# zhaoshan2/pangu-pytorch

Hardware: AMD Instinct MI355X
Metric: forward steps/sec (721x1440x13pl) per MI355X (higher is better)
Workload: dtype f32; 1 GPU; PanguModel fp32 forward, 1 sample/GPU, input (1,5,13,721,1440)+(1,4,721,1440), depths 2-6-6-2, dims 192/384, random-init weights (BASELINE configs[1]); parallelism=dp1

## Files before the change

### include/pangu_hip.h

```cpp
#ifndef PANGU_HIP_H
#define PANGU_HIP_H

#include <stdint.h>

#ifdef __cplusplus
extern "C" {
#endif

#define PANGU_ABI_VERSION 1

#define PANGU_OK 0
#define PANGU_E_SHAPE (-1)
#define PANGU_E_NULL (-2)
#define PANGU_E_DTYPE (-3)
#define PANGU_E_ARG (-4)
#define PANGU_E_RANGE (-5)

#define PANGU_F32 0
#define PANGU_BF16 1

#define PANGU_ACT_NONE 0
#define PANGU_ACT_GELU 1
#define PANGU_ACT_GELU_BWD 2
#define PANGU_ACT_ADD 3
#define PANGU_ACT_GELU_BWD_H 4

typedef void* pangu_stream_t;

int pangu_abi_version(void);
const char* pangu_error_string(int code);


int pangu_window_index_export(pangu_stream_t stream, int32_t* out, int Z, int H, int W, int shifted);

int pangu_window_mask_export(pangu_stream_t stream, float* out, int Z, int H, int W);


int pangu_linear_fwd(pangu_stream_t stream, const float* A, int lda, const float* W, const float* bias,
                     float* C, int ldc, int M, int N, int K, int act, float* aux);

int pangu_split_weight_bf16x3(pangu_stream_t stream, const float* W, int N, int K, void* image);
int pangu_linear_fwd_split(pangu_stream_t stream, const float* A, int lda, const void* image, const float* bias,
                           float* C, int ldc, int M, int N, int K, int act);

int pangu_linear_wgrad(pangu_stream_t stream, const float* dC, int lddc, const float* A, int lda, float* dW,
                       float* db, int M, int N, int K);
int pangu_linear_wgrad_ws(pangu_stream_t stream, const float* dC, int lddc, const float* A, int lda, float* dW,
                          float* db, int M, int N, int K, float* workspace, long long workspace_bytes);


int pangu_lora_wgrad_f32(pangu_stream_t stream, const float* dY, int lddy, const float* X, int ldx, const float* A,
                         const float* B, float* dA, float* dB, int M, int N, int K, int r, float scaling, float* workspace,
                         long long workspace_bytes);
int pangu_lora_wgrad_bf16(pangu_stream_t stream, const void* dY, int lddy, const void* X, int ldx, const float* A, const float* B,
                          float* dA, float* dB, int M, int N, int K, int r, float scaling, float* workspace,
                          long long workspace_bytes);
int pangu_lora_merge_f32(pangu_stream_t stream, const float* W, const float* A, const float* B, float* W_eff, int N, int K,
                         int r, float scaling);


int pangu_lora_dropout_fwd_f32(pangu_stream_t stream, const float* X, int ldx, float* Y, int ldy, const float* A, const float* B,
                               int M, int N, int K, int r, float scaling, double p, unsigned seed, int act, float* H, int ldh);
int pangu_lora_wgrad_dropout_f32(pangu_stream_t stream, const float* dY, int lddy, const float* X, int ldx, const float* A,
                                 const float* B, float* dA, float* dB, float* V, int M, int N, int K, int r, float scaling, double p,
                                 unsigned seed, float* workspace, long long workspace_bytes);
int pangu_lora_dropout_dx_f32(pangu_stream_t stream, float* dX, int lddx, const float* V, const float* A, int M, int K, int r,
                              double p, unsigned seed, const float* pre, int ldpre);


int pangu_lora_dropout_fwd_bf16(pangu_stream_t stream, const void* X, int ldx, void* Y, int ldy, const float* A, const float* B,
                                int M, int N, int K, int r, float scaling, double p, unsigned seed, int act, void* H, int ldh);
int pangu_lora_wgrad_dropout_bf16(pangu_stream_t stream, const void* dY, int lddy, const void* X, int ldx, const float* A,
                                  const float* B, float* dA, float* dB, float* V, int M, int N, int K, int r, float scaling, double p,
                                  unsigned seed, float* workspace, long long workspace_bytes);
int pangu_lora_dropout_dx_bf16(pangu_stream_t stream, void* dX, int lddx, const float* V, const float* A, int M, int K, int r,
                               double p, unsigned seed, const void* pre, int ldpre);


int pangu_window_attn_fwd(pangu_stream_t stream, const float* qkv, const float* qkv_bias, const float* esb,
                          float* out, float* lse, int Z, int H, int W, int C, int heads, int shifted);
int pangu_window_attn_fwd_compact(pangu_stream_t stream, const float* qkv, const float* qkv_bias,
                                  const float* esb_compact, float* out, float* lse, int Z, int H, int W, int C,
                                  int heads, int shifted);

int pangu_attn_windows_fwd(pangu_stream_t stream, const float* qkv, const float* esb, const float* mask,
                           long long mask_lon_stride, float* out, int n_lon, int types, int heads, int C);

int pangu_attn_windows_bwd(pangu_stream_t stream, const float* qkv, const float* esb, const float* mask,
                           long long mask_lon_stride, const float* dout, float* dqkv, float* d_esb, int n_lon, int types,
                           int heads, int C);

int pangu_window_attn_bwd(pangu_stream_t stream, const float* qkv, const float* qkv_bias, const float* esb,
                          const float* out, const float* lse, const float* dout, float* dqkv, float* dqkv_bias,
                          float* d_esb, int Z, int H, int W, int C, int heads, int shifted);


int pangu_ln_residual_fwd(pangu_stream_t stream, const float* y, const float* shortcut, int lds,
                          const float* gamma, const float* beta, float* out, int ldo, float* mean_rstd,
                          int N, int C, float branch_scale);

int pangu_linear_ln_residual_fwd(pangu_stream_t stream, const float* A, int lda, const float* W, const float* bias,
                                 const float* shortcut, int lds, const float* gamma, const float* beta, float* out, int ldo,
                                 int M, int N, int K, float branch_scale);

int pangu_ln_residual_bwd(pangu_stream_t stream, const float* dout, int lddo, const float* y, const float* gamma,
                          float* dy, float* dgamma, float* dbeta, int N, int C, float branch_scale);

int pangu_downsample_ln_fwd(pangu_stream_t stream, const float* x, int ldx, const float* gamma,
                            const float* beta, float* out, float* mean_rstd, int Z, int H, int W, int C);

int pangu_downsample_ln_bwd(pangu_stream_t stream, const float* dout, const float* x, int ldx, const float* gamma,
                            float* dx, float* dgamma, float* dbeta, int Z, int H, int W, int C, const float* dx_add);

int pangu_upsample_ln_fwd(pangu_stream_t stream, const float* y, const float* gamma, const float* beta,
                          float* out, float* mean_rstd, int Z, int H2, int W2, int H, int Co);

int pangu_upsample_ln_bwd(pangu_stream_t stream, const float* dout, const float* y, const float* gamma, float* dy,
                          float* dgamma, float* dbeta, int Z, int H2, int W2, int H, int Co);


int pangu_patch_embed_gather(pangu_stream_t stream, const float* input, const float* input_surface,
                             const float* surface_mean, const float* surface_std, const float* upper_mean,
                             const float* upper_std, const float* maps, const float* const_h,
                             float* a_surface, float* a_upper, int LAT, int LON, int levels_reversed);

int pangu_patch_embed_gather_bwd(pangu_stream_t stream, const float* da_surface, const float* da_upper,
                                 const float* surface_std, const float* upper_std, float* d_input,
                                 float* d_input_surface, int LAT, int LON, int levels_reversed);

int pangu_patch_recover_scatter(pangu_stream_t stream, const float* y_upper, const float* y_surface,
                                float* output, float* output_surface, int LAT, int LON);
int pangu_patch_recover_scatter_denorm(pangu_stream_t stream, const float* y_upper, const float* y_surface, float* output,
                                       float* output_surface, float* phys, float* phys_surface, const float* upper_mean,
                                       const float* upper_std, const float* surface_mean, const float* surface_std, int LAT,
                                       int LON);

int pangu_patch_recover_gather_bwd(pangu_stream_t stream, const float* d_output, const float* d_output_surface,
                                   float* dy_upper, float* dy_surface, int LAT, int LON);


int pangu_lat_weighted_sums(pangu_stream_t stream, const float* pred, const float* target, const float* lat_weight,
                            float* out, int planes, int H, int W);


int pangu_ensemble_perturb_f32(pangu_stream_t stream, float* upper, long long upper_member_stride, float* surface,
                               long long surface_member_stride, int E, int first_member, int H, int W, const float* amplitude,
                               const float* upper_std, const float* surface_std, unsigned int seed, int octaves, int period,
                               float persistence, int control);

int pangu_ensemble_stats_f32(pangu_stream_t stream, const float* members, long long member_stride, int E, const float* target,
                             const float* clim, const float* lat_weight, float* out, float* mean_out, float* std_out,
                             float* workspace, long long workspace_bytes, int planes, int H, int W);


int pangu_linear_fwd_bf16(pangu_stream_t stream, const void* A, int lda, const void* W, const float* bias, void* C,
                          int ldc, int M, int N, int K, int act, void* aux, int out_dtype);

int pangu_window_attn_fwd_bf16(pangu_stream_t stream, const void* qkv, const void* qkv_bias, const void* esb, void* out,
                               float* lse, int Z, int H, int W, int C, int heads, int shifted);

int pangu_window_attn_qkv_fwd_bf16(pangu_stream_t stream, const void* x, int ldx, const void* w_qkv, const float* b_qkv,
                                   const void* esb, void* out, float* lse, int Z, int H, int W, int C, int heads,
                                   int shifted);

int pangu_ln_residual_fwd_bf16(pangu_stream_t stream, const void* y, const void* shortcut, int lds, const float* gamma,
                               const float* beta, void* out, int ldo, int N, int C, float branch_scale);
int pangu_linear_ln_residual_fwd_bf16(pangu_stream_t stream, const void* A, int lda, const void* W, const float* bias,
                                      const void* shortcut, const float* gamma, const float* beta, void* out, int ldo, int M,
                                      int N, int K);
int pangu_mlp_ln_residual_fwd_bf16(pangu_stream_t stream, const void* x, int ldx, const void* w_packed, const float* b1,
                                   const float* b2, const float* gamma, const float* beta, void* out, int ldo, int M,
                                   int C, float branch_scale);
int pangu_mlp_ln_residual_train_fwd_bf16(pangu_stream_t stream, const void* x, int ldx, const void* w_packed,
                                         const float* b1, const float* b2, const float* gamma, const float* beta, void* out,
                                         int ldo, void* pre, int ldp, void* m, int ldm, int M, int C, float branch_scale);
int pangu_linear_gelu_bwd_bf16(pangu_stream_t stream, const void* A, int lda, const void* W, void* dpre, int ldc, int M,
                               int N, int K, const void* pre, void* h);
int pangu_downsample_ln_fwd_bf16(pangu_stream_t stream, const void* x, int ldx, const float* gamma, const float* beta,
                                 void* out, int Z, int H, int W, int C);
int pangu_upsample_ln_fwd_bf16(pangu_stream_t stream, const void* y, const float* gamma, const float* beta, void* out,
                               int Z, int H2, int W2, int H, int Co);

int pangu_patch_embed_gather_bf16(pangu_stream_t stream, const float* input, const float* input_surface,
                                  const float* surface_mean, const float* surface_std, const float* upper_mean,
                                  const float* upper_std, const float* maps, const float* const_h, void* a_surface,
                                  void* a_upper, int LAT, int LON, int levels_reversed);
// ... 70 lines not shown
```

### pangu-pytorch_amd/_lib.py

```python
import ctypes
import os
import re

_HERE = os.path.dirname(os.path.abspath(__file__))
LIB_PATH = os.environ.get("PANGU_HIP_LIB") or os.path.join(_HERE, "libpangu_hip.so")
HEADER_PATH = os.path.join(os.path.dirname(_HERE), "include", "pangu_hip.h")

_c = ctypes
_P, _I, _F = _c.c_void_p, _c.c_int, _c.c_float

SIGNATURES = {
    "pangu_abi_version": [],
    "pangu_error_string": [_I],
    "pangu_window_index_export": [_P, _P, _I, _I, _I, _I],
    "pangu_window_mask_export": [_P, _P, _I, _I, _I],
    "pangu_linear_fwd": [_P, _P, _I, _P, _P, _P, _I, _I, _I, _I, _I, _P],
    "pangu_split_weight_bf16x3": [_P, _P, _I, _I, _P],
    "pangu_linear_fwd_split": [_P, _P, _I, _P, _P, _P, _I, _I, _I, _I, _I],
    "pangu_linear_wgrad": [_P, _P, _I, _P, _I, _P, _P, _I, _I, _I],
    "pangu_linear_wgrad_ws": [_P, _P, _I, _P, _I, _P, _P, _I, _I, _I, _P, _c.c_longlong],
    "pangu_lora_wgrad_f32": [_P, _P, _I, _P, _I, _P, _P, _P, _P, _I, _I, _I, _I, _F, _P, _c.c_longlong],
    "pangu_lora_wgrad_bf16": [_P, _P, _I, _P, _I, _P, _P, _P, _P, _I, _I, _I, _I, _F, _P, _c.c_longlong],
    "pangu_lora_merge_f32": [_P, _P, _P, _P, _P, _I, _I, _I, _F],
    "pangu_lora_dropout_fwd_f32": [_P, _P, _I, _P, _I, _P, _P, _I, _I, _I, _I, _F, _c.c_double, _c.c_uint, _I, _P, _I],
    "pangu_lora_wgrad_dropout_f32": [_P, _P, _I, _P, _I, _P, _P, _P, _P, _P, _I, _I, _I, _I, _F, _c.c_double, _c.c_uint, _P,
                                     _c.c_longlong],
    "pangu_lora_dropout_dx_f32": [_P, _P, _I, _P, _P, _I, _I, _I, _c.c_double, _c.c_uint, _P, _I],
    "pangu_lora_dropout_fwd_bf16": [_P, _P, _I, _P, _I, _P, _P, _I, _I, _I, _I, _F, _c.c_double, _c.c_uint, _I, _P, _I],
    "pangu_lora_wgrad_dropout_bf16": [_P, _P, _I, _P, _I, _P, _P, _P, _P, _P, _I, _I, _I, _I, _F, _c.c_double, _c.c_uint, _P,
                                      _c.c_longlong],
    "pangu_lora_dropout_dx_bf16": [_P, _P, _I, _P, _P, _I, _I, _I, _c.c_double, _c.c_uint, _P, _I],
    "pangu_window_attn_bwd": [_P] * 10 + [_I] * 6,
    "pangu_ln_residual_bwd": [_P, _P, _I, _P, _P, _P, _P, _P, _I, _I, _F],
    "pangu_downsample_ln_bwd": [_P, _P, _P, _I, _P, _P, _P, _P, _I, _I, _I, _I, _P],
    "pangu_upsample_ln_bwd": [_P, _P, _P, _P, _P, _P, _P, _I, _I, _I, _I, _I],
    "pangu_patch_recover_gather_bwd": [_P, _P, _P, _P, _P, _I, _I],
    "pangu_lat_weighted_sums": [_P, _P, _P, _P, _P, _I, _I, _I],
    "pangu_ensemble_perturb_f32": [_P, _P, _c.c_longlong, _P, _c.c_longlong, _I, _I, _I, _I, _P, _P, _P, _c.c_uint, _I, _I, _F, _I],
    "pangu_ensemble_stats_f32": [_P, _P, _c.c_longlong, _I, _P, _P, _P, _P, _P, _P, _P, _c.c_longlong, _I, _I, _I],
    "pangu_linear_fwd_bf16": [_P, _P, _I, _P, _P, _P, _I, _I, _I, _I, _I, _P, _I],
    "pangu_window_attn_fwd_bf16": [_P, _P, _P, _P, _P, _P, _I, _I, _I, _I, _I, _I],
    "pangu_window_attn_qkv_fwd_bf16": [_P, _P, _I, _P, _P, _P, _P, _P, _I, _I, _I, _I, _I, _I],
    "pangu_ln_residual_fwd_bf16": [_P, _P, _P, _I, _P, _P, _P, _I, _I, _I, _F],
    "pangu_linear_ln_residual_fwd_bf16": [_P, _P, _I, _P, _P, _P, _P, _P, _P, _I, _I, _I, _I],
    "pangu_mlp_ln_residual_fwd_bf16": [_P, _P, _I, _P, _P, _P, _P, _P, _P, _I, _I, _I, _F],
    "pangu_mlp_ln_residual_train_fwd_bf16": [_P, _P, _I, _P, _P, _P, _P, _P, _P, _I, _P, _I, _P, _I, _I, _I, _F],
    "pangu_linear_gelu_bwd_bf16": [_P, _P, _I, _P, _P, _I, _I, _I, _I, _P, _P],
    "pangu_downsample_ln_fwd_bf16": [_P, _P, _I, _P, _P, _P, _I, _I, _I, _I],
    "pangu_upsample_ln_fwd_bf16": [_P, _P, _P, _P, _P, _I, _I, _I, _I, _I],
    "pangu_patch_embed_gather_bf16": [_P] * 11 + [_I, _I, _I],
    "pangu_linear_wgrad_bf16": [_P, _P, _I, _P, _I, _P, _P, _I, _I, _I],
    "pangu_linear_wgrad_bf16_ws": [_P, _P, _I, _P, _I, _P, _P, _I, _I, _I, _P, _c.c_longlong],
    "pangu_shadow_refresh_bf16": [_P, _P, _I, _c.c_longlong],
    "pangu_adam_step_multi": [_P, _P, _I, _c.c_longlong] + [_c.c_double] * 5 + [_F, _F],
    "pangu_grad_sumsq_multi": [_P, _P, _I, _c.c_longlong, _P],
    "pangu_grad_clip_state": [_P, _P, _c.c_longlong, _P, _I, _c.c_double, _c.c_double, _I],
    "pangu_adam_step_multi_scaled": [_P, _P, _I, _c.c_longlong] + [_c.c_double] * 5 + [_F, _F, _P],
    "pangu_weighted_l1_loss_blocks": [_I, _I, _c.c_longlong, _I, _c.c_longlong, _I],
    "pangu_weighted_l1_loss_fwd": [_P] * 9 + [_I, _I, _c.c_longlong, _I, _c.c_longlong, _I, _I] + [_P] * 4,
    "pangu_weighted_l1_loss_bwd": [_P] * 10 + [_I, _I, _c.c_longlong, _I, _c.c_longlong, _I, _I] + [_P] * 4,
    "pangu_rollout_l1_seed_bwd": [_P] * 14 + [_I, _I, _c.c_longlong, _I, _c.c_longlong, _I, _I] + [_P] * 4,
    "pangu_fair_crps_loss_blocks": [_I] * 7,
    "pangu_fair_crps_loss_fwd": [_P, _P, _P, _I] + [_P] * 7 + [_I] * 7 + [_P] * 4,
    "pangu_fair_crps_loss_bwd": [_P, _P, _P, _I] + [_P] * 8 + [_I] * 7 + [_P] * 4,
    "pangu_host_copy": [_P, _P, _c.c_longlong, _I],
    "pangu_window_attn_bwd_bf16": [_P] * 10 + [_I] * 6,
    "pangu_ln_residual_bwd_bf16": [_P, _P, _I, _P, _P, _P, _P, _P, _I, _I, _F],
    "pangu_downsample_ln_bwd_bf16": [_P, _P, _P, _I, _P, _P, _P, _P, _I, _I, _I, _I, _P],
    "pangu_upsample_ln_bwd_bf16": [_P, _P, _P, _P, _P, _P, _P, _I, _I, _I, _I, _I],
    "pangu_patch_recover_gather_bwd_bf16": [_P, _P, _P, _P, _P, _I, _I],
    "pangu_window_attn_fwd": [_P, _P, _P, _P, _P, _P, _I, _I, _I, _I, _I, _I],
    "pangu_window_attn_fwd_compact": [_P, _P, _P, _P, _P, _P, _I, _I, _I, _I, _I, _I],
    "pangu_attn_windows_fwd": [_P, _P, _P, _P, _c.c_longlong, _P, _I, _I, _I, _I],
    "pangu_attn_windows_bwd": [_P, _P, _P, _P, _c.c_longlong, _P, _P, _P, _I, _I, _I, _I],
    "pangu_ln_residual_fwd": [_P, _P, _P, _I, _P, _P, _P, _I, _P, _I, _I, _F],
    "pangu_linear_ln_residual_fwd": [_P, _P, _I, _P, _P, _P, _I, _P, _P, _P, _I, _I, _I, _I, _F],
    "pangu_downsample_ln_fwd": [_P, _P, _I, _P, _P, _P, _P, _I, _I, _I, _I],
    "pangu_upsample_ln_fwd": [_P, _P, _P, _P, _P, _P, _I, _I, _I, _I, _I],
    "pangu_patch_embed_gather": [_P] * 11 + [_I, _I, _I],
    "pangu_patch_embed_gather_bwd": [_P] * 7 + [_I, _I, _I],
    "pangu_patch_recover_scatter": [_P, _P, _P, _P, _P, _I, _I],
    "pangu_patch_recover_scatter_denorm": [_P] * 11 + [_I, _I],
    "pangu_traffic_copy": [_P, _P, _P, _c.c_longlong, _I],
}
_RESTYPES = {"pangu_error_string": _c.c_char_p, "pangu_weighted_l1_loss_blocks": _c.c_longlong,
             "pangu_fair_crps_loss_blocks": _c.c_longlong}

_lib = None


def header_functions():
    src = open(HEADER_PATH).read()
    src = re.sub(r"/\*.*?\*/", "", src, flags=re.S)
    return sorted(set(re.findall(r"\b(pangu_[a-z0-9_]+)\s*\(", src)))


def load():
    global _lib
    if _lib is not None:
        return _lib
    if not os.path.exists(LIB_PATH):
        raise RuntimeError(
            f"{LIB_PATH} not found: the HIP extension is not built. Run `python -c 'import __graft_entry__ as g; "
            "g.build()'` (or `make -C pangu-pytorch_amd/csrc`). There is no CPU fallback for this path.")
    import torch
    lib = ctypes.CDLL(LIB_PATH)
    for name, argtypes in SIGNATURES.items():
        fn = getattr(lib, name)
        fn.argtypes = argtypes
        fn.restype = _RESTYPES.get(name, _I)
    if lib.pangu_abi_version() != 1:
        raise RuntimeError("libpangu_hip.so ABI version mismatch")
    _lib = lib
    return lib


def check(rc, what):
    if rc != 0:
        msg = load().pangu_error_string(rc)
        raise RuntimeError(f"{what} failed: {msg.decode() if msg else rc} (code {rc})")
```

### pangu-pytorch_amd/csrc/gemm_f32_split.hip

```cpp
#include "common.h"

namespace {

typedef short bf16x8 __attribute__((ext_vector_type(8)));

constexpr int BM = 128;
constexpr int BN = 192;
constexpr int BK = 16;
constexpr int A_BYTES = BM * 64;
constexpr int PLANE = 2 * BN * 16;
constexpr int B_BYTES = 3 * PLANE;
constexpr int STAGE = A_BYTES + B_BYTES;
constexpr int NSTAGE = 3;
constexpr int A_PIECES = A_BYTES / 1024;
constexpr int PIECES = STAGE / 1024;

__device__ inline int kswz64(int row, int chunk) {
  const int f = (0x78 >> (((row >> 2) & 3) * 2)) & 3;
  return row * 64 + ((chunk ^ f) << 4);
}

__device__ inline void split2(float a, float b, unsigned& hi, unsigned& mid, unsigned& lo) {
  const bf16x2_t h = __builtin_convertvector(f32x2_t{a, b}, bf16x2_t);
  const f32x2_t r1 = f32x2_t{a, b} - __builtin_convertvector(h, f32x2_t);
  const bf16x2_t m = __builtin_convertvector(r1, bf16x2_t);
  const f32x2_t r2 = r1 - __builtin_convertvector(m, f32x2_t);
  hi = __builtin_bit_cast(unsigned, h);
  mid = __builtin_bit_cast(unsigned, m);
  lo = __builtin_bit_cast(unsigned, __builtin_convertvector(r2, bf16x2_t));
}

__device__ inline void split8(const f32x4 c0, const f32x4 c1, bf16x8& hi, bf16x8& mid, bf16x8& lo) {
  unsigned h0, h1, h2, h3, m0, m1, m2, m3, l0, l1, l2, l3;
  split2(c0[0], c0[1], h0, m0, l0);
  split2(c0[2], c0[3], h1, m1, l1);
  split2(c1[0], c1[1], h2, m2, l2);
  split2(c1[2], c1[3], h3, m3, l3);
  hi = __builtin_bit_cast(bf16x8, u32x4{h0, h1, h2, h3});
  mid = __builtin_bit_cast(bf16x8, u32x4{m0, m1, m2, m3});
  lo = __builtin_bit_cast(bf16x8, u32x4{l0, l1, l2, l3});
}

__global__ __launch_bounds__(256) void split_weight_kernel(const float* __restrict__ W, unsigned char* __restrict__ image, int N,
                                                           int K) {
  const int kc = K >> 3;
  const long long t = (long long)blockIdx.x * 256 + threadIdx.x;
  if (t >= (long long)N * kc) return;
  const int n = (int)(t / kc), c = (int)(t - (long long)n * kc);
  const float* src = W + (size_t)n * K + c * 8;
  const f32x4 c0 = *reinterpret_cast<const f32x4*>(src), c1 = *reinterpret_cast<const f32x4*>(src + 4);
  bf16x8 p[3];
  split8(c0, c1, p[0], p[1], p[2]);
  const int nt = n / BN, nl = n - nt * BN, kt = c >> 1, lh = c & 1;
  unsigned char* dst = image + ((size_t)nt * (K / BK) + kt) * B_BYTES + (lh * BN + nl) * 16;
#pragma unroll
  for (int q = 0; q < 3; ++q) *reinterpret_cast<bf16x8*>(dst + q * PLANE) = p[q];
}

template <int ACT, bool HAS_BIAS>
__global__ __launch_bounds__(256, 2) void gemm_f32_split_kernel(const float* __restrict__ A, int lda,
                                                                const unsigned char* __restrict__ image,
                                                                const float* __restrict__ bias, float* __restrict__ C, int ldc,
                                                                int M, int N, int K, int m_tiles, int n_tiles) {
  __shared__ __attribute__((aligned(16))) unsigned char smem[NSTAGE * STAGE];

  const int b = blockIdx.x;
  const int xcd = b & 7, local = b >> 3;
  const int m_tile = (local / n_tiles) * 8 + xcd;
  const int n_tile = local % n_tiles;
  if (m_tile >= m_tiles) return;
  const int m0 = m_tile * BM, n0 = n_tile * BN;

  const int tid = threadIdx.x, lane = tid & 63;
  const int wave = __builtin_amdgcn_readfirstlane(tid >> 6);
  const int wm = wave >> 1, wn = wave & 1;
  const int lr = lane & 31, lh = lane >> 5;
  const int KT = K / BK;

  const __amdgpu_buffer_rsrc_t a_rsrc = __builtin_amdgcn_make_buffer_rsrc(
      const_cast<float*>(A), 0, (int)(((size_t)(M - 1) * lda + K) * sizeof(float)), 0x00020000);
  const __amdgpu_buffer_rsrc_t w_rsrc = __builtin_amdgcn_make_buffer_rsrc(
      const_cast<unsigned char*>(image), 0, (int)((size_t)N * K * 6), 0x00020000);
  unsigned voff_a[2];
#pragma unroll
  for (int i = 0; i < 2; ++i) {
    const int row = 16 * (i * 4 + wave) + (lane >> 2);
    const int f = (0x78 >> (((row >> 2) & 3) * 2)) & 3;
    voff_a[i] = ((unsigned)(m0 + row) * (unsigned)lda + ((lane & 3) ^ f) * 4) * 4u;
  }
  const unsigned voff_w = (unsigned)n_tile * (unsigned)KT * (unsigned)B_BYTES + (unsigned)(wave - A_PIECES) * 1024u + lane * 16;
  auto issue = [&](int kt, int slot) {
    unsigned char* base = smem + slot * STAGE;
#pragma unroll
    for (int i = 0; i < (PIECES + 3) / 4; ++i) {
      const int q = i * 4 + wave;
      auto dst = (__attribute__((address_space(3))) void*)(base + q * 1024);
      if (i < A_PIECES / 4) {
        __builtin_amdgcn_raw_ptr_buffer_load_lds(a_rsrc, dst, 16, (int)voff_a[i], kt * BK * 4, 0, 0);
      } else if (i * 4 + 3 < PIECES || q < PIECES) {
        __builtin_amdgcn_raw_ptr_buffer_load_lds(w_rsrc, dst, 16, (int)(voff_w + i * 4096u), kt * B_BYTES, 0, 0);
      }
    }
  };

  f32x16 acc[2][3];
#pragma unroll
  for (int i = 0; i < 2; ++i)
#pragma unroll
    for (int j = 0; j < 3; ++j)
#pragma unroll
      for (int r = 0; r < 16; ++r) acc[i][j][r] = 0.f;

  int off_a[2][2];
#pragma unroll
  for (int i = 0; i < 2; ++i)
#pragma unroll
    for (int h = 0; h < 2; ++h) off_a[i][h] = kswz64(wm * 64 + i * 32 + lr, 2 * lh + h);
  const int off_w = A_BYTES + (lh * BN + wn * 96 + lr) * 16;

  issue(0, 0);
  if (KT > 1) issue(1, 1);
  int slot = 0;
  for (int kt = 0; kt < KT; ++kt) {
    if (kt + 1 < KT) {
// ... 111 lines not shown
```

### pangu-pytorch_amd/fused.py

```python
import torch

from . import ops, ops_bf16 as ob
from .autograd import DownSampleFn, EarthBlockFn, MlpFn, PatchEmbedFn, PatchRecoverFn, PatchRecoverHalvesFn, UpSampleFn
from . import layers as _layers


def _train_path(module, *tensors):
    if not torch.is_grad_enabled():
        return False
    return any(p.requires_grad for p in module.parameters()) or any(t.requires_grad for t in tensors)


def _stack(outs, B):
    return outs[0].unsqueeze(0) if B == 1 else torch.stack(outs, 0)


def _samples(x):
    if x.shape[0] == 1:
        t = x.reshape(x.shape[1:])
        return [t if t.stride(-1) == 1 and t.dim() == 2 else t.contiguous()]
    return [t.contiguous() for t in x.unbind(0)]


def _tok2d(x):
    B, N, C = x.shape
    if x.stride(2) != 1 or (B > 1 and x.stride(0) != N * x.stride(1)):
        x = x.contiguous()
    return x.as_strided((B * N, C), (x.stride(1), 1), x.storage_offset())


def drop_path_scales(blk):
    dp = blk.drop_path
    if not hasattr(dp, "sample_scale"):
        return 1.0, 1.0
    return dp.sample_scale(blk.training), dp.sample_scale(blk.training)


def embed_constants(statistics, maps, const_h, LAT, LON, dev):
    f32 = lambda t: t.to(device=dev, dtype=torch.float32).contiguous()
    s_mean, s_std, u_mean, u_std = statistics
    return (f32(s_mean).reshape(-1), f32(s_std).reshape(-1), f32(u_mean).reshape(13, 5), f32(u_std).reshape(13, 5),
            f32(maps).reshape(3, 4 * ((LAT + 3) // 4), LON), f32(const_h).reshape(13, LAT, LON))


def concat_halves(x):
    N, C = x.shape[-2:]
    cat = torch.empty((N, 2 * C), dtype=x.dtype, device=x.device)
    return [torch.empty(0, dtype=x.dtype, device=x.device).set_(cat.untyped_storage(), cat.storage_offset() + off, (N, C), (2 * C, 1))
            for off in (0, C)]


def mlp(m, x2d):
    if _train_path(m, x2d) or _drops(m):
        return MlpFn.apply(x2d.contiguous(), _layers.eff_weight(m.linear1), m.linear1.bias, _layers.eff_weight(m.linear2),
                           m.linear2.bias, *_layers.lora_args(m.linear1, m.linear2))
    h = ops.linear(x2d, _layers.eff_weight(m.linear1), m.linear1.bias, act=ops.ACT_GELU)
    return ops.linear(h, _layers.eff_weight(m.linear2), m.linear2.bias)


def _plain_proj(blk, lin, x2, act=ops.ACT_NONE):
    w = _layers.eff_weight(lin)
    if getattr(blk, "split_projections", True):
        image = ops.split_image(lin, w, None if w is lin.weight else ("lora",) + tuple(lin._stamp()))
        if image is not None:
            return ops.linear_split(x2, image, w.shape[0], lin.bias, act=act)
    return ops.linear(x2, w, lin.bias, act=act)


def _block_rows(blk, x2, B, Z, H, W, roll, out=None):
    N, C = x2.shape[0] // B, x2.shape[1]
    att = blk.attention
    s1, s2 = drop_path_scales(blk)
    if s1 != 0.0:
        qkv = _plain_proj(blk, att.linear1, x2)
        esb_c = getattr(att, "_esb_compact", None)
        if esb_c is not None:
            p = att.earth_specific_bias
            if getattr(att, "_esb_compact_stamp", None) != ops.param_stamp(p) or esb_c.device != p.device:
                att._esb_compact = esb_c = None
        cp = esb_c is not None
        esb = esb_c if cp else att.earth_specific_bias[0]
        o = torch.cat([ops.window_attention(qkv[b * N:(b + 1) * N], att.linear1.bias, esb, Z, H, W,
                                            att.head_number, roll, compact=cp) for b in range(B)], 0) if B > 1 else \
            ops.window_attention(qkv, att.linear1.bias, esb, Z, H, W, att.head_number, roll, compact=cp)
        if C in (192, 384):
            x1 = ops.linear_ln_residual(o, _layers.eff_weight(att.linear2), att.linear2.bias, x2, blk.norm1.weight,
                                        blk.norm1.bias, branch_scale=s1)
        else:
            y = ops.linear(o, _layers.eff_weight(att.linear2), att.linear2.bias)
            x1 = ops.ln_residual(y, x2, blk.norm1.weight, blk.norm1.bias, branch_scale=s1)
    else:
        x1 = x2
    if s2 == 0.0:
        return x1 if out is None else out.copy_(x1)
    if C in (192, 384):
        h = _plain_proj(blk, blk.linear.linear1, x1, act=ops.ACT_GELU)
        return ops.linear_ln_residual(h, _layers.eff_weight(blk.linear.linear2), blk.linear.linear2.bias, x1,
                                      blk.norm2.weight, blk.norm2.bias, out=out, branch_scale=s2)
    return ops.ln_residual(mlp(blk.linear, x1), x1, blk.norm2.weight, blk.norm2.bias, out=out, branch_scale=s2)


def _block_rows_bf16(blk, sh, x, Z, H, W, roll, out=None):
    att = blk.attention
    s1, s2 = drop_path_scales(blk)
    C = x.shape[1]
    fuse_proj = x.is_contiguous() and s1 == 1.0 and s2 == 1.0 and C in (192, 384)
    if s1 != 0.0:
        if C in (192, 384):
            o = ob.window_attention_qkv(x, sh.get_lin(att.linear1), att.linear1.bias, sh.get(att.earth_specific_bias),
                                        Z, H, W, att.head_number, roll)
        else:
            qkv = ob.linear(x, sh.get_lin(att.linear1), att.linear1.bias)
            o = ob.window_attention(qkv, sh.get(att.linear1.bias), sh.get(att.earth_specific_bias), Z, H, W,
                                    att.head_number, roll)
        if fuse_proj:
            x1 = ob.linear_ln_residual(o, sh.get_lin(att.linear2), att.linear2.bias, x, blk.norm1.weight, blk.norm1.bias)
        else:
            y = ob.linear(o, sh.get_lin(att.linear2), att.linear2.bias)
            x1 = ob.ln_residual(y, x, blk.norm1.weight, blk.norm1.bias, branch_scale=s1)
    else:
        x1 = x
    if s2 == 0.0:
        return x1 if out is None else out.copy_(x1)
    if C in (192, 384):
        return ob.mlp_ln_residual(x1, sh.get_mlp_lin(blk.linear.linear1, blk.linear.linear2),
                                  blk.linear.linear1.bias, blk.linear.linear2.bias, blk.norm2.weight, blk.norm2.bias,
                                  out=out, branch_scale=s2)
    h = ob.linear(x1, sh.get_lin(blk.linear.linear1), blk.linear.linear1.bias, act=ob.ACT_GELU)
    m = ob.linear(h, sh.get_lin(blk.linear.linear2), blk.linear.linear2.bias)
    return ob.ln_residual(m, x1, blk.norm2.weight, blk.norm2.bias, out=out, branch_scale=s2)


def _drops(layer):
    return layer.training and _layers.dropout_active(layer)


def _infer_arm(layer, sh, infer, *tensors):
    if sh is not None:
        if infer and _drops(layer):
            raise RuntimeError("LoRA adapter dropout in a bf16 train()-mode forward runs on the gradient path only (the inference "
                               "kernels have no materialised projections to correct): call eval() first")
        return infer
    return not (_train_path(layer, *tensors) or _drops(layer))


def sample_block(blk, x, Z, H, W, roll, out=None, sh=None, infer=False):
    if _infer_arm(blk, sh, infer, x):
        return _block_rows(blk, x, 1, Z, H, W, roll, out) if sh is None else _block_rows_bf16(blk, sh, x, Z, H, W, roll, out)
    att = blk.attention
    s1, s2 = drop_path_scales(blk)
    return EarthBlockFn.apply(
        x, blk.norm1.weight, blk.norm1.bias, blk.norm2.weight, blk.norm2.bias,
        _layers.eff_weight(blk.linear.linear1), blk.linear.linear1.bias,
        _layers.eff_weight(blk.linear.linear2), blk.linear.linear2.bias, att.earth_specific_bias,
        _layers.eff_weight(att.linear1), att.linear1.bias, _layers.eff_weight(att.linear2), att.linear2.bias,
        (Z, H, W, att.head_number, bool(roll)), s1, s2, None if out is None else (out,), sh,
        *_layers.lora_args(blk.linear.linear1, blk.linear.linear2, att.linear1, att.linear2))


def _embed_rows(m, inp, inp_surface, consts, levels_reversed, out):
    a_s, a_u = ops.patch_embed_gather(inp, inp_surface, *consts, levels_reversed)
    n_s = a_s.shape[0]
    ops.linear(a_s, m.conv_surface.weight, m.conv_surface.bias, out=out[:n_s])
    ops.linear(a_u, m.conv.weight, m.conv.bias, out=out[n_s:])
    return out


def sample_embed(m, inp, inp_surface, consts, levels_reversed=False, sh=None):
    if sh is None and not _train_path(m, inp, inp_surface):
        LAT, LON = inp.shape[-2], inp.shape[-1]
        x = torch.empty((8 * ((LAT + 3) // 4) * (LON // 4), m.conv.weight.shape[0]), dtype=torch.float32, device=inp.device)
        return _embed_rows(m, inp, inp_surface, consts, levels_reversed, x)
    return PatchEmbedFn.apply(m.conv.weight, m.conv.bias, m.conv_surface.weight, m.conv_surface.bias, inp, inp_surface, *consts,
                              levels_reversed, sh)


def sample_down(m, x, Z, H, W, skip_grad=None, sh=None, infer=False):
    if _infer_arm(m, sh, infer, x):
        if sh is not None:
            return ob.linear(ob.downsample_ln(x, m.norm.weight, m.norm.bias, Z, H, W), sh.get_lin(m.linear))
        return ops.linear(ops.downsample_ln(x, m.norm.weight, m.norm.bias, Z, H, W), _layers.eff_weight(m.linear))
# ... 103 lines not shown
```

### pangu-pytorch_amd/ops.py

```python
import threading
import weakref

import torch

from . import _lib

ACT_NONE, ACT_GELU, ACT_GELU_BWD, ACT_ADD = 0, 1, 2, 3

_timing = None


def timing_start():
    global _timing
    _timing = []


def timing_stop(kind, also=()):
    global _timing
    rec, _timing = _timing or [], None
    torch.cuda.synchronize()

    def agg(tag):
        sel = [(a.elapsed_time(b), w) for k, a, b, w in rec if k == tag]
        return sum(t for t, _ in sel), sum(w for _, w in sel), len(sel)
# ... 259 lines not shown
            linear(a[m0:m1], weight, bias, act, out[m0:m1], aux[m0:m1] if aux is not None else None)
        return out
    with _timed("linear", 2.0 * M * N * K):
        _lib.check(lib.pangu_linear_fwd(_stream(a), ap, lda, wp, bp, op, ldc, M, N, K, act,
                      _chk(aux, "linear.aux") if aux is not None else None), "linear_fwd")
    return out


def split_served(N, K):
    return N % 192 == 0 and K % 16 == 0


def split_weight_image(weight):
    w2 = weight.detach().reshape(weight.shape[0], -1)
    N, K = w2.shape
    if not split_served(N, K) or 6 * N * K >= _U32_BYTES:
        return None
    image = torch.empty((6 * N * K,), dtype=torch.uint8, device=w2.device)
    _lib.check(_lib.load().pangu_split_weight_bf16x3(_stream(w2), _chk(w2, "split.weight"), N, K, image.data_ptr()), "split_weight")
    return image


_split_images = weakref.WeakKeyDictionary()


def split_image(lin, weight, stamp=None):
    if stamp is None:
        stamp = param_stamp(weight)
    hit = _split_images.get(lin)
    if hit is None or hit[0] != stamp:
        require_epoch_hook()
        hit = _split_images[lin] = (stamp, split_weight_image(weight))
    return hit[1]


def drop_split_images(modules):
    for m in modules:
        _split_images.pop(m, None)


def linear_split(a, image, N, bias=None, act=ACT_NONE, out=None):
    lib = _lib.load()
    ap, lda = _rows(a, "linear_split.a")
    M, K = a.shape
    if image.dtype != torch.uint8 or image.numel() != 6 * N * K or not image.is_cuda or not split_served(N, K):
        raise RuntimeError(f"linear_split: image of {image.numel()} bytes does not belong to a served ({N}, {K}) weight")
    bp = _chk(bias, "linear_split.bias") if bias is not None else None
    if out is None:
        out = torch.empty((M, N), dtype=torch.float32, device=a.device)
    op, ldc = _rows(out, "linear_split.out")
    chunks = _row_chunks(M, 4 * lda, 4 * ldc)
    if chunks is not None:
        for m0, m1 in chunks:
            linear_split(a[m0:m1], image, N, bias, act, out[m0:m1])
        return out
    with _timed("linear", 2.0 * M * N * K):
        _lib.check(lib.pangu_linear_fwd_split(_stream(a), ap, lda, image.data_ptr(), bp, op, ldc, M, N, K, act), "linear_fwd_split")
    return out


def linear_ln_residual(a, weight, bias, shortcut, gamma, beta, out=None, branch_scale=1.0):
    lib = _lib.load()
    ap, lda = _rows(a, "linear_ln.a")
    M, K = a.shape
    N = weight.shape[0]
    if weight.shape[1] != K or tuple(shortcut.shape) != (M, N):
        raise RuntimeError(f"linear_ln_residual: a {tuple(a.shape)} weight {tuple(weight.shape)} shortcut {tuple(shortcut.shape)}")
    sp, lds = _rows(shortcut, "linear_ln.shortcut")
    if out is None:
        out = torch.empty((M, N), dtype=torch.float32, device=a.device)
    op, ldo = _rows(out, "linear_ln.out")
    chunks = _row_chunks(M, 4 * lda, 4 * ldo, 4 * lds)
    if chunks is not None:
        for m0, m1 in chunks:
            linear_ln_residual(a[m0:m1], weight, bias, shortcut[m0:m1], gamma, beta, out[m0:m1], branch_scale)
        return out
    with _timed("linear_ln", 2.0 * M * N * K):
        _lib.check(lib.pangu_linear_ln_residual_fwd(
            _stream(a), ap, lda, _chk(weight, "linear_ln.weight"), _chk(bias, "linear_ln.bias") if bias is not None else None,
            sp, lds, _chk(gamma, "gamma"), _chk(beta, "beta"), op, ldo, M, N, K, float(branch_scale)), "linear_ln_residual_fwd")
    return out


_WGRAD_WS_BYTES = 96 << 20
_wgrad_ws = {}


def release_stream_workspaces(stream=None):
    for key in [k for k in _wgrad_ws if stream is None or k[1] == stream.cuda_stream]:
        del _wgrad_ws[key]


def wgrad_workspace(device):
    key = (device, torch.cuda.current_stream(device).cuda_stream)
    ws = _wgrad_ws.get(key)
    if ws is None:
        ws = torch.empty(_WGRAD_WS_BYTES // 4, dtype=torch.float32, device=device)
        _wgrad_ws[key] = ws
    return ws


def linear_wgrad(dc, a, want_bias=True, db_into=None):
    lib = _lib.load()
    ws = wgrad_workspace(dc.device)
    dp, lddc = _rows(dc, "wgrad.dc")
    ap, lda = _rows(a, "wgrad.a")
    M, N = dc.shape
    K = a.shape[1]
    own_db = want_bias and db_into is None
    buf = _zeros((N * K + (N if own_db else 0),), dc.device)
    dw = buf[:N * K].view(N, K)
    db = (buf[N * K:] if own_db else db_into) if want_bias else None
    esz = dc.element_size()
    for m0, m1 in (_row_chunks(M, esz * lddc, esz * lda) or [(0, M)]):
        with _timed("wgrad", 2.0 * (m1 - m0) * N * K):
            _lib.check(lib.pangu_linear_wgrad_ws(_stream(dc), dp + m0 * lddc * esz, lddc, ap + m0 * lda * esz, lda, dw.data_ptr(),
                                                 db.data_ptr() if want_bias else None, m1 - m0, N, K, ws.data_ptr(),
                                                 _WGRAD_WS_BYTES), "linear_wgrad")
    return dw, db


LORA_RANKS = (4, 8, 16, 32)


def lora_wgrad(dy, x, A, B, scaling):
    lib = _lib.load()
    dp, lddy = _rows(dy, "lora_wgrad.dy")
    xp, ldx = _rows(x, "lora_wgrad.x")
    M, N = dy.shape
    K = x.shape[1]
    r = A.shape[0]
    if x.shape[0] != M or tuple(A.shape) != (r, K) or tuple(B.shape) != (N, r):
        raise RuntimeError(f"lora_wgrad: dy {tuple(dy.shape)} x {tuple(x.shape)} A {tuple(A.shape)} B {tuple(B.shape)}")
    ws = wgrad_workspace(dy.device)
    dA = torch.empty((r, K), dtype=torch.float32, device=dy.device)
    dB = torch.empty((N, r), dtype=torch.float32, device=dy.device)
    with _timed("lora_wgrad", 4.0 * M * (K + N)):
        _lib.check(lib.pangu_lora_wgrad_f32(_stream(dy), dp, lddy, xp, ldx, _chk(A, "lora_A"), _chk(B, "lora_B"), dA.data_ptr(),
                                            dB.data_ptr(), M, N, K, r, float(scaling), ws.data_ptr(), _WGRAD_WS_BYTES), "lora_wgrad")
    return dA, dB


def _lora_shapes(what, x, y, A, B):
    M, N = y.shape
    K = x.shape[1]
    r = A.shape[0]
    if x.shape[0] != M or tuple(A.shape) != (r, K) or tuple(B.shape) != (N, r):
        raise RuntimeError(f"{what}: y {tuple(y.shape)} x {tuple(x.shape)} A {tuple(A.shape)} B {tuple(B.shape)}")
    return M, N, K, r


def lora_dropout_fwd(x, y, A, B, scaling, p, seed, act=ACT_NONE, h=None):
    lib = _lib.load()
    xp, ldx = _rows(x, "lora_dropout_fwd.x")
    yp, ldy = _rows(y, "lora_dropout_fwd.y")
    M, N, K, r = _lora_shapes("lora_dropout_fwd", x, y, A, B)
    if act not in (ACT_NONE, ACT_GELU):
        raise RuntimeError(f"lora_dropout_fwd: act {act} (ACT_NONE or ACT_GELU)")
    hp, ldh = (None, 0)
    if act == ACT_GELU:
        if h is None:
            h = torch.empty((M, N), dtype=torch.float32, device=y.device)
        if tuple(h.shape) != (M, N):
            raise RuntimeError(f"lora_dropout_fwd: h {tuple(h.shape)} != {(M, N)}")
        hp, ldh = _rows(h, "lora_dropout_fwd.h")
    with _timed("lora_dropout_fwd", 4.0 * M * (K + 2 * N + (N if act == ACT_GELU else 0))):
# ... 280 lines not shown
```

Baseline: 17.05 forward steps/s.

## Add bf16x3 split-MFMA GEMM fused with LayerNorm residual epilogue

Result: faster. 19.24 forward steps/s, median of 6 (+12.9%).

```diff
diff --git a/include/pangu_hip.h b/include/pangu_hip.h
--- a/include/pangu_hip.h
+++ b/include/pangu_hip.h
@@ -102,6 +102,10 @@
 int pangu_linear_ln_residual_fwd(pangu_stream_t stream, const float* A, int lda, const float* W, const float* bias,
                                  const float* shortcut, int lds, const float* gamma, const float* beta, float* out, int ldo,
                                  int M, int N, int K, float branch_scale);
+
+int pangu_linear_ln_residual_fwd_split(pangu_stream_t stream, const float* A, int lda, const void* image, const float* bias,
+                                       const float* shortcut, int lds, const float* gamma, const float* beta, float* out,
+                                       int ldo, int M, int N, int K, float branch_scale);
 
 int pangu_ln_residual_bwd(pangu_stream_t stream, const float* dout, int lddo, const float* y, const float* gamma,
                           float* dy, float* dgamma, float* dbeta, int N, int C, float branch_scale);
diff --git a/pangu-pytorch_amd/_lib.py b/pangu-pytorch_amd/_lib.py
--- a/pangu-pytorch_amd/_lib.py
+++ b/pangu-pytorch_amd/_lib.py
@@ -75,6 +75,7 @@
     "pangu_attn_windows_bwd": [_P, _P, _P, _P, _c.c_longlong, _P, _P, _P, _I, _I, _I, _I],
     "pangu_ln_residual_fwd": [_P, _P, _P, _I, _P, _P, _P, _I, _P, _I, _I, _F],
     "pangu_linear_ln_residual_fwd": [_P, _P, _I, _P, _P, _P, _I, _P, _P, _P, _I, _I, _I, _I, _F],
+    "pangu_linear_ln_residual_fwd_split": [_P, _P, _I, _P, _P, _P, _I, _P, _P, _P, _I, _I, _I, _I, _F],
     "pangu_downsample_ln_fwd": [_P, _P, _I, _P, _P, _P, _P, _I, _I, _I, _I],
     "pangu_upsample_ln_fwd": [_P, _P, _P, _P, _P, _P, _I, _I, _I, _I, _I],
     "pangu_patch_embed_gather": [_P] * 11 + [_I, _I, _I],
diff --git a/pangu-pytorch_amd/csrc/gemm_f32_split.hip b/pangu-pytorch_amd/csrc/gemm_f32_split.hip
--- a/pangu-pytorch_amd/csrc/gemm_f32_split.hip
+++ b/pangu-pytorch_amd/csrc/gemm_f32_split.hip
@@ -1,45 +1,15 @@
-#include "common.h"
+#include "split_f32.h"
 
 namespace {
 
-typedef short bf16x8 __attribute__((ext_vector_type(8)));
+using namespace pangu_split;
 
 constexpr int BM = 128;
-constexpr int BN = 192;
-constexpr int BK = 16;
+constexpr int BN = W_ROWS;
 constexpr int A_BYTES = BM * 64;
-constexpr int PLANE = 2 * BN * 16;
-constexpr int B_BYTES = 3 * PLANE;
 constexpr int STAGE = A_BYTES + B_BYTES;
-constexpr int NSTAGE = 3;
 constexpr int A_PIECES = A_BYTES / 1024;
 constexpr int PIECES = STAGE / 1024;
-
-__device__ inline int kswz64(int row, int chunk) {
-  const int f = (0x78 >> (((row >> 2) & 3) * 2)) & 3;
-  return row * 64 + ((chunk ^ f) << 4);
-}
-
-__device__ inline void split2(float a, float b, unsigned& hi, unsigned& mid, unsigned& lo) {
-  const bf16x2_t h = __builtin_convertvector(f32x2_t{a, b}, bf16x2_t);
-  const f32x2_t r1 = f32x2_t{a, b} - __builtin_convertvector(h, f32x2_t);
-  const bf16x2_t m = __builtin_convertvector(r1, bf16x2_t);
-  const f32x2_t r2 = r1 - __builtin_convertvector(m, f32x2_t);
-  hi = __builtin_bit_cast(unsigned, h);
-  mid = __builtin_bit_cast(unsigned, m);
-  lo = __builtin_bit_cast(unsigned, __builtin_convertvector(r2, bf16x2_t));
-}
-
-__device__ inline void split8(const f32x4 c0, const f32x4 c1, bf16x8& hi, bf16x8& mid, bf16x8& lo) {
-  unsigned h0, h1, h2, h3, m0, m1, m2, m3, l0, l1, l2, l3;
-  split2(c0[0], c0[1], h0, m0, l0);
-  split2(c0[2], c0[3], h1, m1, l1);
-  split2(c1[0], c1[1], h2, m2, l2);
-  split2(c1[2], c1[3], h3, m3, l3);
-  hi = __builtin_bit_cast(bf16x8, u32x4{h0, h1, h2, h3});
-  mid = __builtin_bit_cast(bf16x8, u32x4{m0, m1, m2, m3});
-  lo = __builtin_bit_cast(bf16x8, u32x4{l0, l1, l2, l3});
-}
 
 __global__ __launch_bounds__(256) void split_weight_kernel(const float* __restrict__ W, unsigned char* __restrict__ image, int N,
                                                            int K) {
diff --git a/pangu-pytorch_amd/csrc/gemm_ln_f32_split.hip b/pangu-pytorch_amd/csrc/gemm_ln_f32_split.hip
--- /dev/null
+++ b/pangu-pytorch_amd/csrc/gemm_ln_f32_split.hip
@@ -0,0 +1,246 @@
+#include "split_f32.h"
+
+namespace {
+
+using namespace pangu_split;
+
+constexpr float LN_EPS = 1e-5f;
+
+__device__ inline float oct_sum(float v) {
+  v += __builtin_bit_cast(float, __builtin_amdgcn_update_dpp(0, __builtin_bit_cast(int, v), 0xB1, 0xF, 0xF, true));
+  v += __builtin_bit_cast(float, __builtin_amdgcn_update_dpp(0, __builtin_bit_cast(int, v), 0x4E, 0xF, 0xF, true));
+  v += __builtin_bit_cast(float, __builtin_amdgcn_update_dpp(0, __builtin_bit_cast(int, v), 0x141, 0xF, 0xF, true));
+  return v;
+}
+
+template <int WMW, int WNW, int NST, bool HAS_BIAS>
+__global__ __launch_bounds__(64 * WMW * WNW, WMW * WNW == 8 ? 1 : 2) void gemm_ln_residual_f32_split_kernel(
+    const float* __restrict__ A, int lda, const unsigned char* __restrict__ image, const float* __restrict__ bias,
+    const float* __restrict__ shortcut, int lds_sc, const float* __restrict__ gamma, const float* __restrict__ beta,
+    float* __restrict__ C, int ldc, int M, int K, float branch_scale) {
+  constexpr int NW = WMW * WNW;
+  constexpr int BM = 64 * WMW;
+  constexpr int BN = 96 * WNW;
+  constexpr int NT = BN / W_ROWS;
+  constexpr int A_BYTES = BM * 64;
+  constexpr int A_PIECES = A_BYTES / 1024;
+  constexpr int STAGE = A_BYTES + NT * B_BYTES;
+  constexpr int PIECES = STAGE / 1024;
+  constexpr int A_IT = A_PIECES / NW;
+  constexpr int IT = (PIECES + NW - 1) / NW;
+  constexpr int REM = PIECES % NW;
+  static_assert(NST == 2 || NST == 3, "ring depth");
+  static_assert(A_PIECES % NW == 0 && BN % W_ROWS == 0, "piece rounds");
+  __shared__ __attribute__((aligned(16))) unsigned char smem[NST * STAGE];
+
+  const int m0 = blockIdx.x * BM;
+  const int tid = threadIdx.x, lane = tid & 63;
+  const int wave = __builtin_amdgcn_readfirstlane(tid >> 6);
+  const int wm = wave / WNW, wn = wave % WNW;
+  const int lr = lane & 31, lh = lane >> 5;
+  const int KT = K / BK;
+
+  const __amdgpu_buffer_rsrc_t a_rsrc = __builtin_amdgcn_make_buffer_rsrc(
+      const_cast<float*>(A), 0, (int)(((size_t)(M - 1) * lda + K) * sizeof(float)), 0x00020000);
+  const __amdgpu_buffer_rsrc_t w_rsrc = __builtin_amdgcn_make_buffer_rsrc(
+      const_cast<unsigned char*>(image), 0, (int)((size_t)BN * K * 6), 0x00020000);
+  unsigned voff_a[A_IT], voff_w[IT - A_IT];
+#pragma unroll
+  for (int i = 0; i < A_IT; ++i) {
+    const int row = 16 * (i * NW + wave) + (lane >> 2);
+    const int f = (0x78 >> (((row >> 2) & 3) * 2)) & 3;
+    voff_a[i] = ((unsigned)(m0 + row) * (unsigned)lda + ((lane & 3) ^ f) * 4) * 4u;
+  }
+#pragma unroll
+  for (int i = A_IT; i < IT; ++i) {
+    const int p = i * NW + wave - A_PIECES;
+    voff_w[i - A_IT] = (unsigned)(p / W_PIECES) * (unsigned)KT * (unsigned)B_BYTES + (unsigned)(p % W_PIECES) * 1024u + lane * 16;
+  }
+  auto issue = [&](int kt, int slot) {
+    unsigned char* base = smem + slot * STAGE;
+#pragma unroll
+    for (int i = 0; i < IT; ++i) {
+      const int q = i * NW + wave;
+      auto dst = (__attribute__((address_space(3))) void*)(base + q * 1024);
+      if (i < A_IT) {
+        __builtin_amdgcn_raw_ptr_buffer_load_lds(a_rsrc, dst, 16, (int)voff_a[i], kt * BK * 4, 0, 0);
+      } else if (i * NW + NW - 1 < PIECES || q < PIECES) {
+        __builtin_amdgcn_raw_ptr_buffer_load_lds(w_rsrc, dst, 16, (int)voff_w[i - A_IT], kt * B_BYTES, 0, 0);
+      }
+    }
+  };
+
+  f32x16 acc[2][3];
+#pragma unroll
+  for (int i = 0; i < 2; ++i)
+#pragma unroll
+    for (int j = 0; j < 3; ++j)
+#pragma unroll
+      for (int r = 0; r < 16; ++r) acc[i][j][r] = 0.f;
+
+  int off_a[2][2];
+#pragma unroll
+  for (int i = 0; i < 2; ++i)
+#pragma unroll
+    for (int h = 0; h < 2; ++h) off_a[i][h] = kswz64(wm * 64 + i * 32 + lr, 2 * lh + h);
+  const int off_w = A_BYTES + (wn >> 1) * B_BYTES + (lh * W_ROWS + (wn & 1) * 96 + lr) * 16;
+
+  issue(0, 0);
+  if (NST == 3 && KT > 1) issue(1, 1);
+  int slot = 0;
+  for (int kt = 0; kt < KT; ++kt) {
+    if (NST == 3 && kt + 1 < KT) {
+      if (REM == 0 || wave < REM) asm volatile("s_waitcnt vmcnt(%0)" ::"n"(IT) : "memory");
+      else asm volatile("s_waitcnt vmcnt(%0)" ::"n"(IT - 1) : "memory");
+    } else {
+      asm volatile("s_waitcnt vmcnt(0)" ::: "memory");
+    }
+    __builtin_amdgcn_s_barrier();
+    asm volatile("" ::: "memory");
+    if (NST == 3) {
+      if (kt + 2 < KT) issue(kt + 2, slot == 0 ? 2 : slot - 1);
+    } else {
+      if (kt + 1 < KT) issue(kt + 1, slot ^ 1);
+    }
+    const unsigned char* St = smem + slot * STAGE;
+    slot = slot == NST - 1 ? 0 : slot + 1;
+
+    bf16x8 bw[3][3];
+#pragma unroll
+    for (int j = 0; j < 3; ++j)
+#pragma unroll
+      for (int p = 0; p < 3; ++p) bw[j][p] = *reinterpret_cast<const bf16x8*>(St + off_w + p * PLANE + j * 512);
+    f32x4 ca[2][2];
+#pragma unroll
+    for (int i = 0; i < 2; ++i)
+#pragma unroll
+      for (int h = 0; h < 2; ++h) ca[i][h] = *reinterpret_cast<const f32x4*>(St + off_a[i][h]);
+    bf16x8 ah[2], am[2], al[2];
+    split8(ca[0][0], ca[0][1], ah[0], am[0], al[0]);
+    auto products = [&](int i) {
+#pragma unroll
+      for (int j = 0; j < 3; ++j) {
+        acc[i][j] = __builtin_amdgcn_mfma_f32_32x32x16_bf16(al[i], bw[j][0], acc[i][j], 0, 0, 0);
+        acc[i][j] = __builtin_amdgcn_mfma_f32_32x32x16_bf16(ah[i], bw[j][2], acc[i][j], 0, 0, 0);
+        acc[i][j] = __builtin_amdgcn_mfma_f32_32x32x16_bf16(am[i], bw[j][1], acc[i][j], 0, 0, 0);
+        acc[i][j] = __builtin_amdgcn_mfma_f32_32x32x16_bf16(am[i], bw[j][0], acc[i][j], 0, 0, 0);
+        acc[i][j] = __builtin_amdgcn_mfma_f32_32x32x16_bf16(ah[i], bw[j][1], acc[i][j], 0, 0, 0);
+        acc[i][j] = __builtin_amdgcn_mfma_f32_32x32x16_bf16(ah[i], bw[j][0], acc[i][j], 0, 0, 0);
+      }
+    };
+    __builtin_amdgcn_sched_barrier(0);
+    products(0);
+    split8(ca[1][0], ca[1][1], ah[1], am[1], al[1]);
+#pragma unroll
+    for (int g = 0; g < 18; ++g) {
+      __builtin_amdgcn_sched_group_barrier(0x008, 1, 0);
+      __builtin_amdgcn_sched_group_barrier(0x002, 3, 0);
+    }
+    __builtin_amdgcn_sched_barrier(0);
+    products(1);
+  }
+  __syncthreads();
+
+  constexpr int EP_LD = 36;
+  float* ep = reinterpret_cast<float*>(smem) + wave * (32 * EP_LD);
+  float* stats = reinterpret_cast<float*>(smem) + NW * (32 * EP_LD);
+  const int er = lane >> 3, ec = (lane & 7) * 4;
+  const __amdgpu_buffer_rsrc_t c_rsrc = __builtin_amdgcn_make_buffer_rsrc(
+      C, 0, (int)(((size_t)(M - 1) * ldc + BN) * sizeof(float)), 0x00020000);
+  const __amdgpu_buffer_rsrc_t s_rsrc = __builtin_amdgcn_make_buffer_rsrc(
+      const_cast<float*>(shortcut), 0, (int)(((size_t)(M - 1) * lds_sc + BN) * sizeof(float)), 0x00020000);
+  constexpr float INV_C = 1.0f / BN;
+#pragma unroll
+  for (int i = 0; i < 2; ++i) {
+    f32x4 y[3][4];
+    float s[4] = {0.f, 0.f, 0.f, 0.f}, q[4] = {0.f, 0.f, 0.f, 0.f};
+#pragma unroll
+    for (int j = 0; j < 3; ++j) {
+      const int col = wn * 96 + j * 32 + ec;
+      f32x4 bv = {0.f, 0.f, 0.f, 0.f};
+      if (HAS_BIAS) bv = *reinterpret_cast<const f32x4*>(bias + col);
+#pragma unroll
+      for (int r = 0; r < 16; ++r) ep[((r & 3) + 8 * (r >> 2) + 4 * lh) * EP_LD + lr] = acc[i][j][r];
+#pragma unroll
+      for (int it = 0; it < 4; ++it) {
+        f32x4 v = *reinterpret_cast<const f32x4*>(&ep[(er + 8 * it) * EP_LD + ec]);
+        v += bv;
+        y[j][it] = v;
+        s[it] += (v[0] + v[1]) + (v[2] + v[3]);
+        q[it] += (v[0] * v[0] + v[1] * v[1]) + (v[2] * v[2] + v[3] * v[3]);
+      }
+    }
+#pragma unroll
+    for (int it = 0; it < 4; ++it) {
+      const float ss = oct_sum(s[it]), qq = oct_sum(q[it]);
+      if ((lane & 7) == 0) {
+        float* st = stats + (((wm * WNW + wn) * 64) + i * 32 + er + 8 * it) * 2;
+        st[0] = ss;
+        st[1] = qq;
+      }
+    }
+    __syncthreads();
+    float mean[4], rstd[4];
+#pragma unroll
+    for (int it = 0; it < 4; ++it) {
+      const int rloc = i * 32 + er + 8 * it;
+      float ts = 0.f, tq = 0.f;
+#pragma unroll
+      for (int w = 0; w < WNW; ++w) {
+        const float* st = stats + ((wm * WNW + w) * 64 + rloc) * 2;
+        ts += st[0];
+        tq += st[1];
+      }
+      mean[it] = ts * INV_C;
+      rstd[it] = rsqrtf(fmaxf(tq * INV_C - mean[it] * mean[it], 0.f) + LN_EPS);
+    }
+#pragma unroll
+    for (int j = 0; j < 3; ++j) {
+      const int col = wn * 96 + j * 32 + ec;
+      const f32x4 gm = *reinterpret_cast<const f32x4*>(gamma + col);
+      const f32x4 bt = *reinterpret_cast<const f32x4*>(beta + col);
+#pragma unroll
+      for (int it = 0; it < 4; ++it) {
+        const unsigned row = (unsigned)(m0 + wm * 64 + i * 32 + er + 8 * it);
+        const f32x4 sc = __builtin_bit_cast(
+            f32x4, __builtin_amdgcn_raw_buffer_load_b128(s_rsrc, (int)((row * (unsigned)lds_sc + (unsigned)col) * 4u), 0, 0));
+        const f32x4 v = sc + branch_scale * ((y[j][it] - mean[it]) * rstd[it] * gm + bt);
+        __builtin_amdgcn_raw_buffer_store_b128(__builtin_bit_cast(u32x4, v), c_rsrc,
+                                               (int)((row * (unsigned)ldc + (unsigned)col) * 4u), 0, 0);
+      }
+    }
+  }
+}
+
+template <int WMW, int WNW, int NST>
+int launch_ln_split(hipStream_t s, const float* A, int lda, const unsigned char* image, const float* bias, const float* shortcut,
+                    int lds, const float* gamma, const float* beta, float* out, int ldo, int M, int K, float branch_scale) {
+  constexpr int BM = 64 * WMW;
+  dim3 g((M + BM - 1) / BM), blk(64 * WMW * WNW);
+  if (bias)
+    hipLaunchKernelGGL((gemm_ln_residual_f32_split_kernel<WMW, WNW, NST, true>), g, blk, 0, s, A, lda, image, bias, shortcut, lds,
+                       gamma, beta, out, ldo, M, K, branch_scale);
+  else
+    hipLaunchKernelGGL((gemm_ln_residual_f32_split_kernel<WMW, WNW, NST, false>), g, blk, 0, s, A, lda, image, bias, shortcut, lds,
+                       gamma, beta, out, ldo, M, K, branch_scale);
+  return pangu_launch_status();
+}
+
+}
+
+extern "C" int pangu_linear_ln_residual_fwd_split(pangu_stream_t stream, const float* A, int lda, const void* image,
+                                                  const float* bias, const float* shortcut, int lds, const float* gamma,
+                                                  const float* beta, float* out, int ldo, int M, int N, int K,
+                                                  float branch_scale) {
+  if (!A || !image || !shortcut || !gamma || !beta || !out) return PANGU_E_NULL;
+  if (M <= 0 || K <= 0 || (K % BK) != 0 || lda < K || (lda & 3) || ldo < N || (ldo & 3) || lds < N || (lds & 3))
+    return PANGU_E_SHAPE;
+  if (N != 192 && N != 384) return PANGU_E_SHAPE;
+  if (!pangu_fits_u32(M, lda, 4) || !pangu_fits_u32(M, ldo, 4) || !pangu_fits_u32(M, lds, 4) ||
+      (long long)N * K * 6 >= 0xFFFFFFFFll)
+    return PANGU_E_RANGE;
+  hipStream_t s = (hipStream_t)stream;
+  const unsigned char* img = reinterpret_cast<const unsigned char*>(image);
+  if (N == 192) return launch_ln_split<2, 2, 3>(s, A, lda, img, bias, shortcut, lds, gamma, beta, out, ldo, M, K, branch_scale);
+  return launch_ln_split<1, 4, 2>(s, A, lda, img, bias, shortcut, lds, gamma, beta, out, ldo, M, K, branch_scale);
+}
diff --git a/pangu-pytorch_amd/csrc/split_f32.h b/pangu-pytorch_amd/csrc/split_f32.h
--- /dev/null
+++ b/pangu-pytorch_amd/csrc/split_f32.h
@@ -0,0 +1,41 @@
+#pragma once
+#include "common.h"
+
+namespace pangu_split {
+
+typedef short bf16x8 __attribute__((ext_vector_type(8)));
+
+constexpr int BK = 16;
+constexpr int W_ROWS = 192;
+constexpr int PLANE = 2 * W_ROWS * 16;
+constexpr int B_BYTES = 3 * PLANE;
+constexpr int W_PIECES = B_BYTES / 1024;
+constexpr int NSTAGE = 3;
+
+__device__ inline int kswz64(int row, int chunk) {
+  const int f = (0x78 >> (((row >> 2) & 3) * 2)) & 3;
+  return row * 64 + ((chunk ^ f) << 4);
+}
+
+__device__ inline void split2(float a, float b, unsigned& hi, unsigned& mid, unsigned& lo) {
+  const bf16x2_t h = __builtin_convertvector(f32x2_t{a, b}, bf16x2_t);
+  const f32x2_t r1 = f32x2_t{a, b} - __builtin_convertvector(h, f32x2_t);
+  const bf16x2_t m = __builtin_convertvector(r1, bf16x2_t);
+  const f32x2_t r2 = r1 - __builtin_convertvector(m, f32x2_t);
+  hi = __builtin_bit_cast(unsigned, h);
+  mid = __builtin_bit_cast(unsigned, m);
+  lo = __builtin_bit_cast(unsigned, __builtin_convertvector(r2, bf16x2_t));
+}
+
+__device__ inline void split8(const f32x4 c0, const f32x4 c1, bf16x8& hi, bf16x8& mid, bf16x8& lo) {
+  unsigned h0, h1, h2, h3, m0, m1, m2, m3, l0, l1, l2, l3;
+  split2(c0[0], c0[1], h0, m0, l0);
+  split2(c0[2], c0[3], h1, m1, l1);
+  split2(c1[0], c1[1], h2, m2, l2);
+  split2(c1[2], c1[3], h3, m3, l3);
+  hi = __builtin_bit_cast(bf16x8, u32x4{h0, h1, h2, h3});
+  mid = __builtin_bit_cast(bf16x8, u32x4{m0, m1, m2, m3});
+  lo = __builtin_bit_cast(bf16x8, u32x4{l0, l1, l2, l3});
+}
+
+}
diff --git a/pangu-pytorch_amd/fused.py b/pangu-pytorch_amd/fused.py
--- a/pangu-pytorch_amd/fused.py
+++ b/pangu-pytorch_amd/fused.py
@@ -65,6 +65,19 @@
         if image is not None:
             return ops.linear_split(x2, image, w.shape[0], lin.bias, act=act)
     return ops.linear(x2, w, lin.bias, act=act)
+
+
+_LN_SPLIT_NOT_DISPATCHED = {(384, 384)}
+
+
+def _ln_proj(blk, lin, x2, shortcut, norm, out=None, branch_scale=1.0):
+    w = _layers.eff_weight(lin)
+    if getattr(blk, "split_projections", True) and tuple(w.shape) not in _LN_SPLIT_NOT_DISPATCHED:
+        image = ops.split_image(lin, w, None if w is lin.weight else ("lora",) + tuple(lin._stamp()))
+        if image is not None:
+            return ops.linear_ln_residual_split(x2, image, w.shape[0], lin.bias, shortcut, norm.weight, norm.bias, out=out,
+                                                branch_scale=branch_scale)
+    return ops.linear_ln_residual(x2, w, lin.bias, shortcut, norm.weight, norm.bias, out=out, branch_scale=branch_scale)
 
 
 def _block_rows(blk, x2, B, Z, H, W, roll, out=None):
@@ -84,8 +97,7 @@
                                             att.head_number, roll, compact=cp) for b in range(B)], 0) if B > 1 else \
             ops.window_attention(qkv, att.linear1.bias, esb, Z, H, W, att.head_number, roll, compact=cp)
         if C in (192, 384):
-            x1 = ops.linear_ln_residual(o, _layers.eff_weight(att.linear2), att.linear2.bias, x2, blk.norm1.weight,
-                                        blk.norm1.bias, branch_scale=s1)
+            x1 = _ln_proj(blk, att.linear2, o, x2, blk.norm1, branch_scale=s1)
         else:
             y = ops.linear(o, _layers.eff_weight(att.linear2), att.linear2.bias)
             x1 = ops.ln_residual(y, x2, blk.norm1.weight, blk.norm1.bias, branch_scale=s1)
@@ -95,8 +107,7 @@
         return x1 if out is None else out.copy_(x1)
     if C in (192, 384):
         h = _plain_proj(blk, blk.linear.linear1, x1, act=ops.ACT_GELU)
-        return ops.linear_ln_residual(h, _layers.eff_weight(blk.linear.linear2), blk.linear.linear2.bias, x1,
-                                      blk.norm2.weight, blk.norm2.bias, out=out, branch_scale=s2)
+        return _ln_proj(blk, blk.linear.linear2, h, x1, blk.norm2, out=out, branch_scale=s2)
     return ops.ln_residual(mlp(blk.linear, x1), x1, blk.norm2.weight, blk.norm2.bias, out=out, branch_scale=s2)
 
 
diff --git a/pangu-pytorch_amd/ops.py b/pangu-pytorch_amd/ops.py
--- a/pangu-pytorch_amd/ops.py
+++ b/pangu-pytorch_amd/ops.py
@@ -365,6 +365,31 @@
     return out
 
 
+def linear_ln_residual_split(a, image, N, bias, shortcut, gamma, beta, out=None, branch_scale=1.0):
+    lib = _lib.load()
+    ap, lda = _rows(a, "linear_ln_split.a")
+    M, K = a.shape
+    if image.dtype != torch.uint8 or image.numel() != 6 * N * K or not image.is_cuda or not split_served(N, K):
+        raise RuntimeError(f"linear_ln_residual_split: image of {image.numel()} bytes does not belong to a served ({N}, {K}) weight")
+    if tuple(shortcut.shape) != (M, N):
+        raise RuntimeError(f"linear_ln_residual_split: a {tuple(a.shape)} weight ({N}, {K}) shortcut {tuple(shortcut.shape)}")
+    sp, lds = _rows(shortcut, "linear_ln_split.shortcut")
+    if out is None:
+        out = torch.empty((M, N), dtype=torch.float32, device=a.device)
+    op, ldo = _rows(out, "linear_ln_split.out")
+    chunks = _row_chunks(M, 4 * lda, 4 * ldo, 4 * lds)
+    if chunks is not None:
+        for m0, m1 in chunks:
+            linear_ln_residual_split(a[m0:m1], image, N, bias, shortcut[m0:m1], gamma, beta, out[m0:m1], branch_scale)
+        return out
+    with _timed("linear_ln", 2.0 * M * N * K):
+        _lib.check(lib.pangu_linear_ln_residual_fwd_split(
+            _stream(a), ap, lda, image.data_ptr(), _chk(bias, "linear_ln_split.bias") if bias is not None else None,
+            sp, lds, _chk(gamma, "gamma"), _chk(beta, "beta"), op, ldo, M, N, K, float(branch_scale)),
+            "linear_ln_residual_fwd_split")
+    return out
+
+
 _WGRAD_WS_BYTES = 96 << 20
 _wgrad_ws = {}
 
```
